# cvxopt/cvxopt

Hardware: NVIDIA H100
Metric: kkt_factor_solve_gflops_fp64 (higher is better)
Workload: dtype f64

## Files before the change

cvxopt_b200/csrc/chol.cu:

```cuda
#include "common.cuh"
#include <cstdlib>

namespace cvxb {

namespace {

constexpr int PB = 8;
constexpr int SP = 12;
constexpr int LDM = NB + 4;
constexpr int POTF2_SMEM = (NB * LDM + NB * SP + 4 * 80) * 8;

template <int PAT>
__device__ __forceinline__ void sym_update(double (&acc)[4][8][2], const double *Ma, const double *Mb) {
#pragma unroll 2
    for (int kk = 0; kk < NB / 4; ++kk) {
        double a[4], bfr[8];
#pragma unroll
        for (int cf = 0; cf < 4; ++cf) a[cf] = -Ma[cf * 8 + kk * 4 * LDM];
#pragma unroll
        for (int rf = 0; rf < 8; ++rf) bfr[rf] = Mb[rf * 8 + kk * 4 * LDM];
#pragma unroll
        for (int mf = 0; mf < 2; ++mf)
#pragma unroll
            for (int rf = 0; rf < 8; ++rf) {
                if (PAT == 1 && rf < 2 * mf) continue;
                if (PAT == 2 && rf < 4 + 2 * mf) continue;
                dmma16x8x4(acc[2 * mf][rf][0], acc[2 * mf][rf][1], acc[2 * mf + 1][rf][0], acc[2 * mf + 1][rf][1],
                           a[2 * mf], a[2 * mf + 1], bfr[rf]);
            }
    }
}

__global__ void __launch_bounds__(256, 1)
potf2_inv_kernel(double *A, long long lda, int jb, double *inv, double *invT, int *info, int joff,
                 long long sA, long long sInv, const double *Tprev, long long ldt,
                 const double *invprev, unsigned long long *trace) {
    extern __shared__ __align__(16) double sm[];
    if (trace && threadIdx.x == 0) {
        unsigned long long t; asm volatile("mov.u64 %0, %%globaltimer;" : "=l"(t)); trace[0] = t;
    }
#define CVXB_STAMP(SLOT)                                                                    \
    if (trace && threadIdx.x == 0) {                                                        \
        unsigned long long t_; asm volatile("mov.u64 %0, %%globaltimer;" : "=l"(t_));       \
        trace[8 * 2048 + (SLOT)] = t_;                                                      \
    }
    A += (long long)blockIdx.x * sA; inv += (long long)blockIdx.x * sInv;
    invT += (long long)blockIdx.x * sInv; info += blockIdx.x;
    double *M = sm;
    double *P = M + NB * LDM;
    double *Dw = P + NB * SP;
    const int tid = threadIdx.x, lane = tid & 31, warp = tid >> 5;
    const int role = (0x72640531 >> (warp * 4)) & 7;
    const int wr = role & 1, wc = role >> 1;
    const int g4 = lane >> 2, t4 = lane & 3;

    double acc[4][8][2];
    if (Tprev != nullptr) {
#pragma unroll
        for (int cf = 0; cf < 4; ++cf)
#pragma unroll
            for (int rf = 0; rf < 8; ++rf) acc[cf][rf][0] = acc[cf][rf][1] = 0.0;
        const int kkmax = (wc + 1) * 8;
        {
            const bool v16 = ((ldt & 1) == 0) && ((reinterpret_cast<uintptr_t>(Tprev) & 15) == 0);
            if (v16) {
                for (int q = tid; q < NB * NB / 2; q += 256) {
                    const int c = q >> 6, r = (q & 63) * 2;
                    const int nb = (r + 1 < jb) ? 16 : (r < jb ? 8 : 0);
                    cp_async16(M + r + c * LDM, nb ? Tprev + r + (long long)c * ldt : Tprev, nb);
                }
            } else {
                for (int q = tid; q < NB * NB; q += 256) {
                    const int c = q >> 7, r = q & 127;
                    cp_async8(M + r + c * LDM, (r < jb) ? Tprev + r + (long long)c * ldt : Tprev, (r < jb) ? 8 : 0);
                }
            }
            cp_async_commit();
        }
        const double *ip = invprev + (wc * 32 + g4) + t4 * NB;
        double a0[4];
#pragma unroll
        for (int cf = 0; cf < 4; ++cf) a0[cf] = ip[cf * 8];
        cp_async_wait<0>();
        __syncthreads();
        const double *tq = M + (wr * 64 + g4) + t4 * LDM;
#pragma unroll 2
        for (int kk = 0; kk < kkmax; ++kk) {
            double a[4], bfr[8];
#pragma unroll
            for (int cf = 0; cf < 4; ++cf) a[cf] = a0[cf];
            if (kk + 1 < kkmax) {
#pragma unroll
                for (int cf = 0; cf < 4; ++cf) a0[cf] = ip[cf * 8 + (kk + 1) * 4 * NB];
            }
#pragma unroll
            for (int rf = 0; rf < 8; ++rf) bfr[rf] = tq[rf * 8 + kk * 4 * LDM];
#pragma unroll
            for (int mf = 0; mf < 2; ++mf)
#pragma unroll
                for (int rf = 0; rf < 8; ++rf)
                    dmma16x8x4(acc[2 * mf][rf][0], acc[2 * mf][rf][1], acc[2 * mf + 1][rf][0],
                               acc[2 * mf + 1][rf][1], a[2 * mf], a[2 * mf + 1], bfr[rf]);
        }
        __syncthreads();
#pragma unroll
        for (int cf = 0; cf < 4; ++cf)
#pragma unroll
            for (int rf = 0; rf < 8; ++rf)
#pragma unroll
                for (int e = 0; e < 2; ++e)
                    M[(wr * 64 + rf * 8 + t4 * 2 + e) + (wc * 32 + cf * 8 + g4) * LDM] = acc[cf][rf][e];
    }
    CVXB_STAMP(0)
#pragma unroll
    for (int cf = 0; cf < 4; ++cf)
#pragma unroll
        for (int rf = 0; rf < 8; ++rf)
#pragma unroll
            for (int e = 0; e < 2; ++e) {
                const int r = wr * 64 + rf * 8 + t4 * 2 + e, c = wc * 32 + cf * 8 + g4;
                double v = (r == c) ? 1.0 : 0.0;
                if (r < jb && c < jb && r >= c) v = A[r + (long long)c * lda];
                acc[cf][rf][e] = v;
            }
    __syncthreads();
    CVXB_STAMP(4)
    if (Tprev != nullptr) {
        const int d = wc - 2 * wr;
        const double *Ma = M + (wc * 32 + g4) + t4 * LDM;
        const double *Mb = M + (wr * 64 + g4) + t4 * LDM;
        if (d < 0) sym_update<0>(acc, Ma, Mb);
        else if (d == 0) sym_update<1>(acc, Ma, Mb);
        else if (d == 1) sym_update<2>(acc, Ma, Mb);
        __syncthreads();
    }
    CVXB_STAMP(1)
#pragma unroll 1
    for (int t = 0; t < NB / PB; ++t) {
      {
        const int c0 = t * PB;
        if (wc == (t >> 2)) {
#define CVXB_PUBLISH(CF)                                                          \
    _Pragma("unroll") for (int rf = 0; rf < 8; ++rf)                              \
        _Pragma("unroll") for (int e = 0; e < 2; ++e)                             \
            P[(wr * 64 + rf * 8 + t4 * 2 + e) * SP + g4] = acc[CF][rf][e];
            switch (t & 3) {
                case 0: CVXB_PUBLISH(0) break;
                case 1: CVXB_PUBLISH(1) break;
                case 2: CVXB_PUBLISH(2) break;
                default: CVXB_PUBLISH(3) break;
            }
#undef CVXB_PUBLISH
        }
        __syncthreads();
        if (warp == 0 && lane == 0) {
            double a[PB][PB];
#pragma unroll
            for (int i = 0; i < PB; ++i)
#pragma unroll
                for (int k = 0; k <= i; ++k) a[i][k] = P[(c0 + i) * SP + k];
            bool bad = false;
#pragma unroll
            for (int j = 0; j < PB; ++j) {
                const double piv = a[j][j];
                if (!(piv > 0.0) && !bad) {
                    atomicCAS(info, 0, joff + c0 + j + 1);
                    bad = true;
                }
                const double rs = rsqrt(piv);
                a[j][j] = piv * rs;
                Dw[64 + j] = rs;
#pragma unroll
                for (int i = j + 1; i < PB; ++i) a[i][j] *= rs;
#pragma unroll
                for (int k = j + 1; k < PB; ++k)
#pragma unroll
                    for (int i = k; i < PB; ++i) a[i][k] -= a[i][j] * a[k][j];
            }
#pragma unroll
            for (int i = 0; i < PB; ++i)
#pragma unroll
                for (int k = 0; k < PB; ++k) Dw[i * 8 + k] = (k <= i) ? a[i][k] : 0.0;
        }
        if (warp < 4) asm volatile("bar.sync 1, 128;" ::: "memory");
        if (warp < 4) {
            const double *D = Dw;
            const int r = warp * 32 + lane;
            double x[PB];
            if (r >= c0 + PB) {
#pragma unroll
                for (int j = 0; j < PB; ++j) x[j] = P[r * SP + j];
#pragma unroll
                for (int j = 0; j < PB; ++j) {
                    double v = x[j];
#pragma unroll
                    for (int k = 0; k < j; ++k) v -= x[k] * D[j * 8 + k];
                    x[j] = v * D[64 + j];
                }
            } else if (r >= c0) {
#pragma unroll
                for (int j = 0; j < PB; ++j) x[j] = (j <= r - c0) ? D[(r - c0) * 8 + j] : 0.0;
            } else {
#pragma unroll
                for (int j = 0; j < PB; ++j) x[j] = 0.0;
            }
#pragma unroll
            for (int j = 0; j < PB; ++j) P[r * SP + j] = x[j];
        }
        __syncthreads();
        if (wr * 8 + 7 > t && wc * 4 + 3 > t) {
            double a[4][2], bfr[8][2];
#pragma unroll
            for (int kk = 0; kk < 2; ++kk) {
#pragma unroll
                for (int cf = 0; cf < 4; ++cf) a[cf][kk] = -P[(wc * 32 + cf * 8 + g4) * SP + kk * 4 + t4];
#pragma unroll
                for (int rf = 0; rf < 8; ++rf) bfr[rf][kk] = P[(wr * 64 + rf * 8 + g4) * SP + kk * 4 + t4];
            }
#pragma unroll
            for (int mf = 0; mf < 2; ++mf) {
                if (wc * 4 + 2 * mf + 1 <= t) continue;
#pragma unroll
                for (int rf = 0; rf < 8; ++rf) {
                    dmma16x8x4(acc[2 * mf][rf][0], acc[2 * mf][rf][1], acc[2 * mf + 1][rf][0], acc[2 * mf + 1][rf][1],
                               a[2 * mf][0], a[2 * mf + 1][0], bfr[rf][0]);
                    dmma16x8x4(acc[2 * mf][rf][0], acc[2 * mf][rf][1], acc[2 * mf + 1][rf][0], acc[2 * mf + 1][rf][1],
                               a[2 * mf][1], a[2 * mf + 1][1], bfr[rf][1]);
                }
            }
        }
        for (int e = tid; e < NB * PB; e += 256) {
            const int r = e & (NB - 1), j = e >> 7;
            const double v = P[r * SP + j];
            M[r + (c0 + j) * LDM] = v;
            if (r >= c0 + j && r < jb && c0 + j < jb) A[r + (long long)(c0 + j) * lda] = v;
        }
        __syncthreads();
      }
    }

    CVXB_STAMP(2)
    {
        const int blk = warp * 2 + (lane >> 4);
        const int j = lane & 15;
        const int o = blk * PB;
        double x[PB];
        if (j < PB) {
#pragma unroll
            for (int i = 0; i < PB; ++i) {
                double v = (i == j) ? 1.0 : 0.0;
#pragma unroll
                for (int k = 0; k < i; ++k)
                    if (k >= j) v -= M[(o + i) + (o + k) * LDM] * x[k];
                x[i] = (i >= j) ? v / M[(o + i) + (o + i) * LDM] : 0.0;
            }
        }
        __syncwarp();
        if (j < PB) {
#pragma unroll
            for (int i = 0; i < PB; ++i) M[(o + i) + (o + j) * LDM] = x[i];
        }
    }
    __syncthreads();
    for (int s = PB; s < NB; s <<= 1) {
        const int sb = s / PB;
        const int tp = sb * sb;
        const int ntiles = (NB / (2 * s)) * tp;
#pragma unroll 1
        for (int phase = 0; phase < 2; ++phase) {
            for (int base = warp * 4; base < ntiles; base += 32) {
                double c[4][2];
                int oo[4], ti[4], tj[4];
#pragma unroll
                for (int u = 0; u < 4; ++u) {
                    const int idx = min(base + u, ntiles - 1);
                    const int pr = idx / tp, loc = idx - pr * tp;
                    ti[u] = loc % sb; tj[u] = loc / sb; oo[u] = pr * 2 * s;
                    c[u][0] = c[u][1] = 0.0;
                }
                for (int kb = 0; kb < sb; ++kb) {
#pragma unroll
                    for (int u = 0; u < 4; ++u) {
                        const bool live = phase == 0 ? (kb >= tj[u]) : (kb <= ti[u]);
                        if (!live) continue;
                        const int o = oo[u];
#pragma unroll
                        for (int kk = 0; kk < 2; ++kk) {
                            const int k = kb * 8 + kk * 4 + t4;
                            double af, bf;
                            if (phase == 0) {
                                af = M[(o + s + ti[u] * 8 + g4) + (o + k) * LDM];
                                bf = M[(o + k) + (o + tj[u] * 8 + g4) * LDM];
                            } else {
                                af = M[(o + s + ti[u] * 8 + g4) + (o + s + k) * LDM];
                                bf = M[(o + k) + (o + s + tj[u] * 8 + g4) * LDM];
                            }
                            dmma(c[u][0], c[u][1], af, bf);
                        }
                    }
                }
#pragma unroll
                for (int u = 0; u < 4; ++u) {
                    if (base + u >= ntiles) continue;
                    const int o = oo[u];
                    if (phase == 0) {
                        M[(o + ti[u] * 8 + g4) + (o + s + tj[u] * 8 + t4 * 2) * LDM] = c[u][0];
                        M[(o + ti[u] * 8 + g4) + (o + s + tj[u] * 8 + t4 * 2 + 1) * LDM] = c[u][1];
                    } else {
                        M[(o + s + ti[u] * 8 + g4) + (o + tj[u] * 8 + t4 * 2) * LDM] = -c[u][0];
                        M[(o + s + ti[u] * 8 + g4) + (o + tj[u] * 8 + t4 * 2 + 1) * LDM] = -c[u][1];
                    }
                }
            }
            __syncthreads();
        }
    }
    CVXB_STAMP(3)
    for (int e = tid; e < NB * NB; e += 256) {
        int i = e & (NB - 1), k = e >> 7;
        inv[e] = (i >= k) ? M[i + k * LDM] : 0.0;
        invT[e] = (k >= i) ? M[k + i * LDM] : 0.0;
    }
    if (trace && threadIdx.x == 0) {
        unsigned long long t; asm volatile("mov.u64 %0, %%globaltimer;" : "=l"(t)); trace[1] = t;
    }
}

constexpr int TR_CH = 32;
constexpr int TR_R = 5;
constexpr int TRSV_SMEM = (TR_R * NB * TR_CH + 4 * NB + 32 * 129) * 8;

template <bool TRANS, bool VEC>
__global__ void __launch_bounds__(256, 1)
trsv_kernel(int n, const double *__restrict__ L, long long ldl, const double *__restrict__ inv,
            const double *__restrict__ invT, double *b, int *flags, int epoch, long long sL,
            long long sInv, long long sb) {
    extern __shared__ __align__(16) double sm[];
    {
        const long long pb = blockIdx.y;
        L += pb * sL; inv += pb * sInv; invT += pb * sInv; b += pb * sb;
        flags += pb * ((n + NB - 1) / NB);
    }
    double *ring = sm;
    double *xs = ring + TR_R * NB * TR_CH;
    double *part = xs + NB;
    double *tvec = part + 2 * NB;
    double *part2 = tvec + NB;
    const int nblk = (n + NB - 1) / NB;
    const int tid = threadIdx.x, lane = tid & 31, warp = tid >> 5;
    const int bi = TRANS ? (nblk - 1 - (int)blockIdx.x) : (int)blockIdx.x;
    const int i0 = bi * NB;
    const int ni = min(NB, n - i0);
    const int r = tid & (NB - 1), half = tid >> 7;

    double ireg[64];
    {
        const double *ip = (TRANS ? invT : inv) + (long long)bi * NB * NB + r + (long long)(half * 64) * NB;
#pragma unroll
        for (int k = 0; k < 64; ++k) ireg[k] = ip[k * NB];
    }

    const double bown = (tid < ni) ? b[i0 + tid] : 0.0;
    const int nb_dep = TRANS ? (nblk - 1 - bi) : bi;
    const int nchunks = nb_dep * (NB / TR_CH);
    auto issue = [&](int q) {
        const int jj = q / (NB / TR_CH), cc = q % (NB / TR_CH);
        const int j = TRANS ? (nblk - 1 - jj) : jj;
        double *dst = ring + (q % TR_R) * (NB * TR_CH);
        const double *src;
        int nrows, ncols;
        if (!TRANS) { src = L + i0 + (long long)(j * NB + cc * TR_CH) * ldl; nrows = ni; ncols = TR_CH; }
        else { src = L + (long long)j * NB + (long long)(i0 + cc * TR_CH) * ldl; nrows = min(NB, n - j * NB); ncols = min(TR_CH, ni - cc * TR_CH); }
        if (VEC) {
#pragma unroll
            for (int it = 0; it < 8; ++it) {
                const int e = tid + it * 256;
                const int c = e >> 6, rr = (e & 63) * 2;
                const int rem = nrows - rr;
                const int bytes = (c < ncols) ? (rem >= 2 ? 16 : (rem == 1 ? 8 : 0)) : 0;
                cp_async16(dst + c * NB + rr, bytes ? (src + rr + (long long)c * ldl) : L, bytes);
            }
        } else {
#pragma unroll
            for (int it = 0; it < 16; ++it) {
                const int e = tid + it * 256;
                const int c = e >> 7, rr = e & 127;
                const int bytes = (c < ncols && rr < nrows) ? 8 : 0;
                cp_async8(dst + c * NB + rr, bytes ? (src + rr + (long long)c * ldl) : L, bytes);
            }
        }
    };
#pragma unroll
    for (int q = 0; q < TR_R - 1; ++q) {
        if (q < nchunks) issue(q);
        cp_async_commit();
    }

    double acc = 0.0;
    double accc[16];
#pragma unroll
    for (int q = 0; q < 16; ++q) accc[q] = 0.0;

    for (int jj = 0; jj < nb_dep; ++jj) {
        const int j = TRANS ? (nblk - 1 - jj) : jj;
        if (tid == 0) while (ld_acquire(flags + j) != epoch) { }
        __syncthreads();
        if (tid < NB) xs[tid] = (j * NB + tid < n) ? __ldcg(b + j * NB + tid) : 0.0;
#pragma unroll
        for (int cc = 0; cc < NB / TR_CH; ++cc) {
            const int q = jj * (NB / TR_CH) + cc;
            cp_async_wait<TR_R - 2>();
            __syncthreads();
            {
                const int nq = q + TR_R - 1;
                if (nq < nchunks) issue(nq);
                cp_async_commit();
            }
            const double *ch = ring + (q % TR_R) * (NB * TR_CH);
            if (!TRANS) {
#pragma unroll
                for (int c = 0; c < 16; ++c)
                    acc += ch[(half * 16 + c) * NB + r] * xs[cc * TR_CH + half * 16 + c];
            } else {
#pragma unroll
                for (int qc = 0; qc < 4; ++qc) {
                    const double *col = ch + (warp * 4 + qc) * NB;
                    double a = 0.0;
#pragma unroll
                    for (int rr = 0; rr < 4; ++rr) a += col[lane + rr * 32] * xs[lane + rr * 32];
                    accc[cc * 4 + qc] += a;
                }
            }
        }
    }
    cp_async_wait<0>();
    __syncthreads();
    if (!TRANS) {
        part[half * NB + r] = acc;
        __syncthreads();
        if (tid < NB) tvec[tid] = (tid < ni) ? (bown - part[tid] - part[NB + tid]) : 0.0;
        __syncthreads();
    } else {
#pragma unroll
        for (int q = 0; q < 16; ++q) {
            const int c = (q >> 2) * TR_CH + warp * 4 + (q & 3);
            part2[lane * 129 + c] = accc[q];
        }
        __syncthreads();
        if (tid < NB) {
            double sacc = 0.0;
#pragma unroll 8
            for (int l = 0; l < 32; ++l) sacc += part2[l * 129 + tid];
            tvec[tid] = (tid < ni) ? (bown - sacc) : 0.0;
        }
        __syncthreads();
    }
    double a2 = 0.0;
#pragma unroll
    for (int k = 0; k < 64; ++k) a2 += ireg[k] * tvec[half * 64 + k];
    part[half * NB + r] = a2;
    __syncthreads();
    if (tid < ni) b[i0 + tid] = part[tid] + part[NB + tid];
    __threadfence();
    __syncthreads();
    if (tid == 0) st_release(flags + bi, epoch);
}

std::atomic<int> g_trsv_epoch{0};

}

int chol_work_create(CholWork &w) {
    int least = 0, greatest = 0;
    CVXB_CUDA(cudaDeviceGetStreamPriorityRange(&least, &greatest));
    CVXB_CUDA(cudaStreamCreateWithPriority(&w.panel_stream, cudaStreamNonBlocking, greatest));
    CVXB_CUDA(cudaStreamCreateWithPriority(&w.trsm_stream, cudaStreamNonBlocking, greatest));
    CVXB_CUDA(cudaStreamCreateWithPriority(&w.update_stream, cudaStreamNonBlocking, least));
    CVXB_CUDA(cudaEventCreateWithFlags(&w.ev_end_t, cudaEventDisableTiming));
    CVXB_CUDA(cudaEventCreateWithFlags(&w.ev_start, cudaEventDisableTiming));
    CVXB_CUDA(cudaEventCreateWithFlags(&w.ev_end_p, cudaEventDisableTiming));
    CVXB_CUDA(cudaEventCreateWithFlags(&w.ev_end_u, cudaEventDisableTiming));
    CVXB_TRY(w.d_info.alloc(1));
    CVXB_CUDA(cudaMemset(w.d_info.p, 0, sizeof(int)));
    CVXB_TRY(w.d_flags.alloc(4096));
    CVXB_CUDA(cudaMemset(w.d_flags.p, 0, 4096 * sizeof(int)));
    CVXB_TRY(w.splitk_ws.alloc(dmma_gemm_splitk_ws_doubles()));
    CVXB_CUDA(cudaFuncSetAttribute(potf2_inv_kernel, cudaFuncAttributeMaxDynamicSharedMemorySize,
                                   POTF2_SMEM));
    CVXB_CUDA(cudaFuncSetAttribute(trsv_kernel<true, true>, cudaFuncAttributeMaxDynamicSharedMemorySize, TRSV_SMEM));
    CVXB_CUDA(cudaFuncSetAttribute(trsv_kernel<true, false>, cudaFuncAttributeMaxDynamicSharedMemorySize, TRSV_SMEM));
    CVXB_CUDA(cudaFuncSetAttribute(trsv_kernel<false, true>, cudaFuncAttributeMaxDynamicSharedMemorySize, TRSV_SMEM));
    CVXB_CUDA(cudaFuncSetAttribute(trsv_kernel<false, false>, cudaFuncAttributeMaxDynamicSharedMemorySize, TRSV_SMEM));
    return 0;
}

CholWork::~CholWork() {
    for (cudaStream_t s : {panel_stream, update_stream, trsm_stream}) if (s) cudaStreamDestroy(s);
    for (auto &g : graphs) if (g.exec) cudaGraphExecDestroy(g.exec);
    for (cudaEvent_t e : {ev_end_t, ev_start, ev_end_p, ev_end_u}) if (e) cudaEventDestroy(e);
    for (auto *v : {&ev_dg, &ev_tr, &ev_c0, &ev_r})
        for (cudaEvent_t e : *v) cudaEventDestroy(e);
}

static int potrf_enqueue(int n, double *A, int lda, double *inv, CholWork &w, cudaStream_t st) {
    if (n <= 0) return 0;
    const int nblk = (n + NB - 1) / NB;
    if (w.panel_rows < n) {
        for (auto &g : w.graphs) if (g.exec) cudaGraphExecDestroy(g.exec);
        w.graphs.clear();
        for (DevBuf<double> &pb : w.panel) pb.reset();
        const int rows = (n + 1) & ~1;
        for (DevBuf<double> &pb : w.panel) CVXB_TRY(pb.alloc((size_t)rows * NB));
        w.panel_rows = rows;
    }
    while ((int)w.ev_dg.size() < nblk) {
        cudaEvent_t e[4];
        for (int i = 0; i < 4; ++i) CVXB_CUDA(cudaEventCreateWithFlags(&e[i], cudaEventDisableTiming));
        w.ev_dg.push_back(e[0]); w.ev_tr.push_back(e[1]); w.ev_c0.push_back(e[2]); w.ev_r.push_back(e[3]);
    }
    if (getenv("CVXB_TRACE") && !w.trace.p) CVXB_TRY(w.trace.alloc(8 * 4096));
    unsigned long long *trace = w.trace.p;
    if (trace) CVXB_CUDA(cudaMemsetAsync(trace, 0, 8 * 4096 * sizeof(unsigned long long), st));
    const int ldw = w.panel_rows;
    const int panel_tiles = NB / dmma_gemm_tile_cols();
    cudaStream_t D = w.panel_stream, T = w.trsm_stream, U = w.update_stream;
    CVXB_CUDA(cudaMemsetAsync(w.d_info.p, 0, sizeof(int), st));
    CVXB_CUDA(cudaEventRecord(w.ev_start, st));
    CVXB_CUDA(cudaStreamWaitEvent(D, w.ev_start, 0));
    CVXB_CUDA(cudaStreamWaitEvent(T, w.ev_start, 0));
    CVXB_CUDA(cudaStreamWaitEvent(U, w.ev_start, 0));
    int last_r = -1;
    int prev_r = -1;
    for (int jb = 0; jb < nblk; ++jb) {
        const int j = jb * NB;
        const int wj = (n - j < NB) ? (n - j) : NB;
        const int m = n - j - wj;
        double *Ajj = A + j + (long long)j * lda;
        double *invj = inv + (long long)jb * NB * NB;
        double *invTj = inv + (long long)(nblk + jb) * NB * NB;
        double *Wp = w.panel[jb & 1].p;
        if (jb >= 2) {
            CVXB_CUDA(cudaStreamWaitEvent(D, w.ev_c0[jb - 2], 0));
            const int rd = (last_r <= jb - 2) ? last_r : prev_r;
            if (rd >= 0) CVXB_CUDA(cudaStreamWaitEvent(D, w.ev_r[rd], 0));
        }
        const double *Tprev = jb > 0 ? A + j + (long long)(j - NB) * lda : nullptr;
        const double *invprev = jb > 0 ? inv + (long long)(jb - 1) * NB * NB : nullptr;
        potf2_inv_kernel<<<1, 256, POTF2_SMEM, D>>>(Ajj, lda, wj, invj, invTj, w.d_info.p, j, 0, 0, Tprev,
                                                     lda, invprev, trace ? trace + 8 * jb : nullptr);
        count_launch();
        CVXB_LAUNCH_CHECK();
        CVXB_CUDA(cudaEventRecord(w.ev_dg[jb], D));
        auto copy_back_prev = [&]() -> int {
            if (jb == 0) return 0;
            const int jp = j - NB, mp = n - j;
            CVXB_CUDA(cudaMemcpy2DAsync(A + j + (long long)jp * lda, (size_t)lda * sizeof(double),
                                        w.panel[(jb - 1) & 1].p, (size_t)ldw * sizeof(double),
                                        (size_t)mp * sizeof(double), NB, cudaMemcpyDeviceToDevice, T));
            return 0;
        };
        if (m <= 0) {
            CVXB_CUDA(cudaStreamWaitEvent(T, w.ev_dg[jb], 0));
            CVXB_TRY(copy_back_prev());
            break;
        }
        double *A21 = Ajj + wj;
        double *A22 = A21 + (long long)wj * lda;
        CVXB_CUDA(cudaStreamWaitEvent(T, w.ev_dg[jb], 0));
        if (prev_r >= 0) CVXB_CUDA(cudaStreamWaitEvent(T, w.ev_r[prev_r], 0));
        {
            GemmDesc g;
            g.M = m; g.N = wj; g.K = wj;
            g.X = A21; g.ldx = lda; g.x_kmajor = false;
            g.Y = invj; g.ldy = NB; g.y_kmajor = false;
            g.C = Wp; g.ldc = ldw;
            g.trace = trace ? trace + 8 * jb + 2 : nullptr;
            CVXB_TRY(dmma_gemm(g, T));
        }
        CVXB_CUDA(cudaEventRecord(w.ev_tr[jb], T));
        if (last_r >= 0) CVXB_CUDA(cudaStreamWaitEvent(T, w.ev_r[last_r], 0));
        const int wn = (m < NB) ? m : NB;
        if (m > wn) {
            GemmDesc c;
            c.M = m - wn; c.N = wn; c.K = wj;
            c.X = Wp + wn; c.Y = Wp;
            c.ldx = ldw; c.x_kmajor = false;
            c.ldy = ldw; c.y_kmajor = false;
            c.D = A22 + wn; c.ldd = lda; c.C = A22 + wn; c.ldc = lda;
            c.alpha = -1.0; c.beta = 1.0;
            c.trace = trace ? trace + 8 * jb + 4 : nullptr;
            CVXB_TRY(dmma_gemm(c, T));
        }
        CVXB_CUDA(cudaEventRecord(w.ev_c0[jb], T));
        CVXB_TRY(copy_back_prev());
        if (m > NB) {
            CVXB_CUDA(cudaStreamWaitEvent(U, w.ev_tr[jb], 0));
            GemmDesc u;
            u.M = m; u.N = m; u.K = wj;
            u.X = Wp; u.ldx = ldw; u.x_kmajor = false;
            u.Y = Wp; u.ldy = ldw; u.y_kmajor = false;
            u.D = A22; u.ldd = lda; u.C = A22; u.ldc = lda;
            u.alpha = -1.0; u.beta = 1.0; u.lower_only = true;
            u.ct_begin = panel_tiles; u.ct_end = 1 << 30;
            u.trace = trace ? trace + 8 * jb + 6 : nullptr;
            CVXB_TRY(dmma_gemm(u, U));
            CVXB_CUDA(cudaEventRecord(w.ev_r[jb], U));
            prev_r = last_r;
            last_r = jb;
        }
    }
    CVXB_CUDA(cudaEventRecord(w.ev_end_p, D));
    CVXB_CUDA(cudaEventRecord(w.ev_end_u, U));
    CVXB_CUDA(cudaEventRecord(w.ev_end_t, T));
    CVXB_CUDA(cudaStreamWaitEvent(st, w.ev_end_p, 0));
    CVXB_CUDA(cudaStreamWaitEvent(st, w.ev_end_u, 0));
    CVXB_CUDA(cudaStreamWaitEvent(st, w.ev_end_t, 0));
    return 0;
}

int potrf_lower(int n, double *A, int lda, double *inv, CholWork &w, cudaStream_t st) {
    if (n <= 0) return 0;
    if (w.graph_failed || n > 4096) return potrf_enqueue(n, A, lda, inv, w, st);
    CholWork::GraphEntry *ent = nullptr;
    for (auto &g : w.graphs)
        if (g.n == n && g.A == A && g.lda == lda && g.inv == inv) { ent = &g; break; }
    if (ent && ent->exec) {
        CVXB_CUDA(cudaGraphLaunch(ent->exec, st));
        count_launch(ent->launches);
        return 0;
    }
    if (!ent) {
        if (w.graphs.size() >= 4) {
            for (auto &g : w.graphs) if (g.exec) cudaGraphExecDestroy(g.exec);
            w.graphs.clear();
        }
        CholWork::GraphEntry g;
        g.n = n; g.A = A; g.lda = lda; g.inv = inv;
        w.graphs.push_back(g);
        return potrf_enqueue(n, A, lda, inv, w, st);
    }
    const unsigned long long l0 = g_launches.load();
    if (cudaStreamBeginCapture(st, cudaStreamCaptureModeRelaxed) != cudaSuccess) {
        cudaGetLastError();
        w.graph_failed = true;
        return potrf_enqueue(n, A, lda, inv, w, st);
    }
    const int rc = potrf_enqueue(n, A, lda, inv, w, st);
    cudaGraph_t graph = nullptr;
    const cudaError_t ce = cudaStreamEndCapture(st, &graph);
    const int captured = (int)(g_launches.load() - l0);
    g_launches.fetch_sub((unsigned long long)captured);
    if (rc != 0 || ce != cudaSuccess || !graph) {
        cudaGetLastError();
        if (graph) cudaGraphDestroy(graph);
        w.graph_failed = true;
        return potrf_enqueue(n, A, lda, inv, w, st);
    }
    cudaGraphExec_t exec = nullptr;
    if (cudaGraphInstantiate(&exec, graph, 0) != cudaSuccess || !exec) {
        cudaGetLastError();
        cudaGraphDestroy(graph);
        w.graph_failed = true;
        return potrf_enqueue(n, A, lda, inv, w, st);
    }
    cudaGraphDestroy(graph);
    ent->exec = exec;
    ent->launches = captured;
    CVXB_CUDA(cudaGraphLaunch(exec, st));
    count_launch(captured);
    return 0;
}

int trsv_lower(int n, const double *L, int ldl, const double *inv, double *b, bool trans,
               CholWork &w, cudaStream_t st, int batch, long long sL, long long sInv, long long sb) {
    if (n <= 0 || batch <= 0) return 0;
    const int nblk = (n + NB - 1) / NB;
    const size_t nflags = (size_t)nblk * batch;
    if (nflags > w.d_flags.n) {
        w.d_flags.reset();
        CVXB_TRY(w.d_flags.alloc(nflags));
        CVXB_CUDA(cudaMemset(w.d_flags.p, 0, nflags * sizeof(int)));
    }
    const int epoch = g_trsv_epoch.fetch_add(1) + 1;
    const double *invT = inv + (long long)nblk * NB * NB;
    const bool vec = ((uintptr_t)L % 16 == 0) && (ldl % 2 == 0) && (batch == 1 || sL % 2 == 0);
    dim3 grid(nblk, batch);
#define TRSV_LAUNCH(T, V) trsv_kernel<T, V><<<grid, 256, TRSV_SMEM, st>>>(n, L, ldl, inv, invT, b, w.d_flags.p, epoch, sL, sInv, sb)
    if (trans) { if (vec) TRSV_LAUNCH(true, true); else TRSV_LAUNCH(true, false); }
    else       { if (vec) TRSV_LAUNCH(false, true); else TRSV_LAUNCH(false, false); }
#undef TRSV_LAUNCH
    count_launch();
    CVXB_LAUNCH_CHECK();
    return 0;
}

int potrs_lower(int n, const double *L, int ldl, const double *inv, double *b, CholWork &w,
                cudaStream_t st, int batch, long long sL, long long sInv, long long sb) {
    CVXB_TRY(trsv_lower(n, L, ldl, inv, b, false, w, st, batch, sL, sInv, sb));
    CVXB_TRY(trsv_lower(n, L, ldl, inv, b, true, w, st, batch, sL, sInv, sb));
    return 0;
}

namespace {
__global__ void copy2d_batched_kernel(const double *src, long long lds, long long ssrc, double *dst,
                                      long long ldd, long long sdst, int rows, int cols) {
    const long long pb = blockIdx.z;
    const int r = blockIdx.x * blockDim.x + threadIdx.x, c = blockIdx.y;
    if (r < rows && c < cols) dst[pb * sdst + r + (long long)c * ldd] = src[pb * ssrc + r + (long long)c * lds];
}
}

int potrf_lower_batched(int n, double *A, int lda, long long sA, double *inv, long long sInv,
                        int batch, int *d_info, double *panel, int ldw, cudaStream_t st) {
    if (n <= 0 || batch <= 0) return 0;
    const int nblk = (n + NB - 1) / NB;
    CVXB_CUDA(cudaMemsetAsync(d_info, 0, (size_t)batch * sizeof(int), st));
    const long long sW = (long long)ldw * NB;
    for (int jb = 0; jb < nblk; ++jb) {
        const int j = jb * NB;
        const int wj = (n - j < NB) ? (n - j) : NB;
        const int m = n - j - wj;
        double *Ajj = A + j + (long long)j * lda;
        double *invj = inv + (long long)jb * NB * NB;
        double *invTj = inv + (long long)(nblk + jb) * NB * NB;
        potf2_inv_kernel<<<batch, 256, POTF2_SMEM, st>>>(Ajj, lda, wj, invj, invTj, d_info, j, sA, sInv, nullptr, 0,
                                                        nullptr, nullptr);
        count_launch();
        CVXB_LAUNCH_CHECK();
        if (m <= 0) break;
        double *A21 = Ajj + wj;
        double *A22 = A21 + (long long)wj * lda;
        GemmDesc g;
        g.M = m; g.N = wj; g.K = wj;
        g.X = A21; g.ldx = lda; g.x_kmajor = false; g.sX = sA;
        g.Y = invj; g.ldy = NB; g.y_kmajor = false; g.sY = sInv;
        g.C = panel; g.ldc = ldw; g.sC = sW; g.batch = batch;
        CVXB_TRY(dmma_gemm(g, st));
        GemmDesc u;
        u.M = m; u.N = m; u.K = wj;
        u.X = panel; u.ldx = ldw; u.x_kmajor = false; u.sX = sW;
        u.Y = panel; u.ldy = ldw; u.y_kmajor = false; u.sY = sW;
        u.D = A22; u.ldd = lda; u.sD = sA; u.C = A22; u.ldc = lda; u.sC = sA;
        u.alpha = -1.0; u.beta = 1.0; u.lower_only = true; u.batch = batch;
        CVXB_TRY(dmma_gemm(u, st));
        dim3 cg((m + 255) / 256, wj, batch);
        copy2d_batched_kernel<<<cg, 256, 0, st>>>(panel, ldw, sW, A21, lda, sA, m, wj);
        count_launch();
        CVXB_LAUNCH_CHECK();
    }
    return 0;
}

}
```

cvxopt_b200/csrc/common.cuh:

```cuda
#pragma once
#include <cuda_runtime.h>
#include <cstdio>
#include <cstdint>
#include <cstring>
#include <string>
#include <vector>
#include <atomic>
#include <mutex>
#include "../../include/cvxopt_b200.h"

namespace cvxb {

void set_error(const char *fmt, ...);
extern std::atomic<unsigned long long> g_launches;
inline void count_launch(int n = 1) { g_launches.fetch_add((unsigned long long)n, std::memory_order_relaxed); }

struct DeviceOnce {
    std::atomic<unsigned long long> done{0};
    unsigned long long pending() {
        int d = 0;
        cudaGetDevice(&d);
        const unsigned long long bit = 1ull << (d & 63);
        return (done.load(std::memory_order_acquire) & bit) ? 0ull : bit;
    }
    void mark(unsigned long long bit) { done.fetch_or(bit, std::memory_order_release); }
};

#define CVXB_CUDA(expr)                                                            \
    do {                                                                           \
        cudaError_t _e = (expr);                                                   \
        if (_e != cudaSuccess) {                                                   \
            cvxb::set_error("%s:%d: %s -> %s", __FILE__, __LINE__, #expr,          \
                            cudaGetErrorString(_e));                               \
            return CVXB_E_CUDA;                                                    \
        }                                                                          \
    } while (0)

#define CVXB_TRY(expr)                                                             \
    do {                                                                           \
        int _r = (expr);                                                           \
        if (_r != 0) return _r;                                                    \
    } while (0)

#define CVXB_LAUNCH_CHECK()                                                        \
    do {                                                                           \
        cudaError_t _e = cudaGetLastError();                                       \
        if (_e != cudaSuccess) {                                                   \
            cvxb::set_error("%s:%d: kernel launch -> %s", __FILE__, __LINE__,      \
                            cudaGetErrorString(_e));                               \
            return CVXB_E_CUDA;                                                    \
        }                                                                          \
    } while (0)

cudaError_t tmp_malloc_bytes(void **p, size_t bytes);
void tmp_free(void *p);
void tmp_cache_release();
template <class T> inline cudaError_t tmp_malloc(T **p, size_t bytes) { return tmp_malloc_bytes(reinterpret_cast<void **>(p), bytes); }

template <class T> struct Scratch {
    T *p = nullptr;
    Scratch() = default;
    Scratch(const Scratch &) = delete;
    Scratch &operator=(const Scratch &) = delete;
    ~Scratch() { tmp_free(p); }
    int alloc(size_t n) {
        CVXB_CUDA(tmp_malloc(&p, (n ? n : 1) * sizeof(T)));
        return 0;
    }
};

struct Staged {
    double *dev = nullptr, *host = nullptr; size_t n = 0; bool owned = false;
    Staged() = default;
    Staged(const Staged &) = delete;
    Staged &operator=(const Staged &) = delete;
    ~Staged() { if (owned) tmp_free(dev); }
    int in(const double *src, size_t count, int space, cudaStream_t st, bool upload = true) {
        n = count; host = const_cast<double *>(src);
        if (space == CVXB_DEVICE) { dev = host; return 0; }
        CVXB_CUDA(tmp_malloc(&dev, (n ? n : 1) * sizeof(double)));
        owned = true;
        if (n && upload) CVXB_CUDA(cudaMemcpyAsync(dev, src, n * sizeof(double), cudaMemcpyHostToDevice, st));
        return 0;
    }
    int out(cudaStream_t st) {
        if (owned && n) CVXB_CUDA(cudaMemcpyAsync(host, dev, n * sizeof(double), cudaMemcpyDeviceToHost, st));
        return 0;
    }
};

extern std::atomic<unsigned long long> g_device_bytes;

template <class T> struct DevBuf {
    T *p = nullptr;
    size_t n = 0;
    DevBuf() = default;
    DevBuf(const DevBuf &) = delete;
    DevBuf &operator=(const DevBuf &) = delete;
    DevBuf(DevBuf &&o) noexcept : p(o.p), n(o.n) { o.p = nullptr; o.n = 0; }
    DevBuf &operator=(DevBuf &&o) noexcept {
        if (this != &o) { reset(); p = o.p; n = o.n; o.p = nullptr; o.n = 0; }
        return *this;
    }
    ~DevBuf() { reset(); }
    cudaError_t try_alloc(size_t count) {
        reset();
        const size_t bytes = count * sizeof(T);
        cudaError_t e = cudaMalloc(&p, bytes);
        if (e == cudaErrorMemoryAllocation) { cudaGetLastError(); tmp_cache_release(); e = cudaMalloc(&p, bytes); }
        if (e != cudaSuccess) { cudaGetLastError(); p = nullptr; return e; }
        n = count;
        g_device_bytes.fetch_add(bytes, std::memory_order_relaxed);
        return cudaSuccess;
    }
    int alloc(size_t count) {
        const cudaError_t e = try_alloc(count);
        if (e == cudaSuccess) return 0;
        set_error("cudaMalloc(%zu bytes) -> %s", count * sizeof(T), cudaGetErrorString(e));
        return e == cudaErrorMemoryAllocation ? CVXB_E_NOMEM : CVXB_E_CUDA;
    }
    void reset() {
        if (!p) return;
        cudaFree(p);
        g_device_bytes.fetch_sub(n * sizeof(T), std::memory_order_relaxed);
        p = nullptr;
        n = 0;
    }
};

bool coop_launch_fits(const void *kernel, int threads, long long ctas);

constexpr int kNumSMs = 132;
constexpr int NB = 128;

#ifdef __CUDACC__
__device__ __forceinline__ void dmma(double &d0, double &d1, double a, double b) {
    asm volatile("mma.sync.aligned.m8n8k4.row.col.f64.f64.f64.f64 {%0,%1}, {%2}, {%3}, {%0,%1};"
                 : "+d"(d0), "+d"(d1)
                 : "d"(a), "d"(b));
}
__device__ __forceinline__ void dmma16x8x4(double &d0, double &d1, double &d2, double &d3, double a0, double a1,
                                           double b) {
    asm volatile("mma.sync.aligned.m16n8k4.row.col.f64.f64.f64.f64 {%0,%1,%2,%3}, {%4,%5}, {%6}, {%0,%1,%2,%3};"
                 : "+d"(d0), "+d"(d1), "+d"(d2), "+d"(d3)
                 : "d"(a0), "d"(a1), "d"(b));
}

__device__ __forceinline__ uint32_t smem_u32(const void *p) {
    return (uint32_t)__cvta_generic_to_shared(p);
}
__device__ __forceinline__ void cp_async16(void *smem, const void *gmem, int src_bytes) {
    asm volatile("cp.async.cg.shared.global [%0], [%1], 16, %2;" ::"r"(smem_u32(smem)), "l"(gmem),
                 "r"(src_bytes));
}
__device__ __forceinline__ void cp_async8(void *smem, const void *gmem, int src_bytes) {
    asm volatile("cp.async.ca.shared.global [%0], [%1], 8, %2;" ::"r"(smem_u32(smem)), "l"(gmem),
                 "r"(src_bytes));
}
__device__ __forceinline__ void cp_async_commit() { asm volatile("cp.async.commit_group;"); }
template <int N>
__device__ __forceinline__ void cp_async_wait() {
    asm volatile("cp.async.wait_group %0;" ::"n"(N));
}

__device__ __forceinline__ void mbar_init(uint64_t *bar, int count) {
    asm volatile("mbarrier.init.shared::cta.b64 [%0], %1;" ::"r"(smem_u32(bar)), "r"(count));
}
__device__ __forceinline__ void mbar_expect_tx(uint64_t *bar, uint32_t bytes) {
    asm volatile("mbarrier.arrive.expect_tx.shared::cta.b64 _, [%0], %1;" ::"r"(smem_u32(bar)), "r"(bytes)
                 : "memory");
}
__device__ __forceinline__ void mbar_arrive(uint64_t *bar) {
    asm volatile("mbarrier.arrive.shared::cta.b64 _, [%0];" ::"r"(smem_u32(bar)) : "memory");
}
__device__ __forceinline__ void mbar_wait(uint64_t *bar, uint32_t parity) {
    asm volatile(
        "{\n\t.reg .pred p;\n\t"
        "WAIT_%=:\n\t"
        "mbarrier.try_wait.parity.shared::cta.b64 p, [%0], %1;\n\t"
        "@p bra DONE_%=;\n\t"
        "bra WAIT_%=;\n\t"
        "DONE_%=:\n\t}" ::"r"(smem_u32(bar)), "r"(parity)
        : "memory");
}
__device__ __forceinline__ void bulk_g2s(void *dst, const void *src, uint32_t bytes, uint64_t *bar) {
    asm volatile(
        "cp.async.bulk.shared::cluster.global.mbarrier::complete_tx::bytes [%0], [%1], %2, [%3];"
        ::"r"(smem_u32(dst)), "l"(src), "r"(bytes), "r"(smem_u32(bar))
        : "memory");
}
__device__ __forceinline__ void tma_load_1d(void *dst, const void *map, int c0, uint64_t *bar) {
    asm volatile(
        "cp.async.bulk.tensor.1d.shared::cluster.global.tile.mbarrier::complete_tx::bytes [%0], [%1, {%2}], [%3];"
        ::"r"(smem_u32(dst)), "l"(map), "r"(c0), "r"(smem_u32(bar))
        : "memory");
}
__device__ __forceinline__ void tma_load_2d(void *dst, const void *map, int c0, int c1, uint64_t *bar) {
    asm volatile(
        "cp.async.bulk.tensor.2d.shared::cluster.global.tile.mbarrier::complete_tx::bytes [%0], [%1, {%2, %3}], [%4];"
        ::"r"(smem_u32(dst)), "l"(map), "r"(c0), "r"(c1), "r"(smem_u32(bar))
        : "memory");
}

__device__ __forceinline__ double warp_sum(double v) {
#pragma unroll
    for (int o = 16; o > 0; o >>= 1) v += __shfl_xor_sync(0xffffffffu, v, o);
    return v;
}
__device__ __forceinline__ double warp_min(double v) {
#pragma unroll
    for (int o = 16; o > 0; o >>= 1) v = fmin(v, __shfl_xor_sync(0xffffffffu, v, o));
    return v;
}
__device__ __forceinline__ double block_sum(double v, double *sh) {
    v = warp_sum(v);
    const int lane = threadIdx.x & 31, warp = threadIdx.x >> 5;
    __syncthreads();
    if (lane == 0) sh[warp] = v;
    __syncthreads();
    double t = (threadIdx.x < (blockDim.x >> 5)) ? sh[threadIdx.x] : 0.0;
    if (warp == 0) t = warp_sum(t);
    if (threadIdx.x == 0) sh[0] = t;
    __syncthreads();
    const double r = sh[0];
    __syncthreads();
    return r;
}
__device__ __forceinline__ double block_min(double v, double *sh) {
    v = warp_min(v);
    const int lane = threadIdx.x & 31, warp = threadIdx.x >> 5;
    __syncthreads();
    if (lane == 0) sh[warp] = v;
    __syncthreads();
    double t = (threadIdx.x < (blockDim.x >> 5)) ? sh[threadIdx.x] : INFINITY;
    if (warp == 0) t = warp_min(t);
    if (threadIdx.x == 0) sh[0] = t;
    __syncthreads();
    const double r = sh[0];
    __syncthreads();
    return r;
}
__device__ __forceinline__ int ld_acquire(const int *p) {
    int v;
    asm volatile("ld.acquire.gpu.global.s32 %0, [%1];" : "=r"(v) : "l"(p) : "memory");
    return v;
}
__device__ __forceinline__ void st_release(int *p, int v) {
    asm volatile("st.release.gpu.global.s32 [%0], %1;" ::"l"(p), "r"(v) : "memory");
}
#endif

struct GemmDesc {
    int M = 0, N = 0, K = 0;
    const double *X = nullptr; int ldx = 0; bool x_kmajor = false;
    const double *Y = nullptr; int ldy = 0; bool y_kmajor = false;
    const double *w = nullptr;
    const double *D = nullptr; int ldd = 0;
    double *C = nullptr; int ldc = 0;
    double alpha = 1.0, beta = 0.0;
    bool lower_only = false;
    int ct_begin = 0, ct_end = 1 << 30;
    int batch = 1;
    long long sX = 0, sY = 0, sW = 0, sD = 0, sC = 0;
    double *splitk_ws = nullptr;
    unsigned long long *trace = nullptr;
};
int dmma_gemm(const GemmDesc &g, cudaStream_t st);
size_t dmma_gemm_splitk_ws_doubles();
int dmma_gemm_tile_cols();

size_t ozaki_workspace_bytes(int n, int m, int S);
int ozaki_mode();
bool ozaki_use(int mode, int n, int m, DevBuf<char> &work);
void ozaki_time_mma(cudaEvent_t a, cudaEvent_t b);
int ozaki_syrk(int n, int m, const double *A, long long lda, const double *d, const double *D,
               long long ldd, double beta, double *C, long long ldc, int S, int layout, void *work,
               cudaStream_t st);

struct CholWork {
    cudaStream_t panel_stream = nullptr;
    cudaStream_t trsm_stream = nullptr;
    cudaStream_t update_stream = nullptr;
    cudaEvent_t ev_end_t = nullptr;
    std::vector<cudaEvent_t> ev_dg, ev_tr, ev_c0, ev_r;
    DevBuf<unsigned long long> trace;
    struct GraphEntry {
        int n = 0, lda = 0, launches = 0;
        const void *A = nullptr, *inv = nullptr;
        cudaGraphExec_t exec = nullptr;
    };
    std::vector<GraphEntry> graphs;
    bool graph_failed = false;
    cudaEvent_t ev_start = nullptr, ev_end_p = nullptr, ev_end_u = nullptr;
    DevBuf<int> d_info;
    DevBuf<int> d_flags;
    DevBuf<double> splitk_ws;
    DevBuf<double> panel[2];
    int panel_rows = 0;
    ~CholWork();
};
int chol_work_create(CholWork &w);
int potrf_lower(int n, double *A, int lda, double *inv, CholWork &w, cudaStream_t st);
int potrs_lower(int n, const double *L, int ldl, const double *inv, double *b, CholWork &w,
                cudaStream_t st, int batch = 1, long long sL = 0, long long sInv = 0,
                long long sb = 0);
int trsv_lower(int n, const double *L, int ldl, const double *inv, double *b, bool trans,
               CholWork &w, cudaStream_t st, int batch = 1, long long sL = 0, long long sInv = 0,
               long long sb = 0);
int potrf_lower_batched(int n, double *A, int lda, long long sA, double *inv, long long sInv,
                        int batch, int *d_info, double *panel, int ldw, cudaStream_t st);
int trsm_lower_left(int n, const double *L, long long ldl, const double *inv, double *B, long long ldb, int ncols,
                    cudaStream_t st, int batch = 1, long long sL = 0, long long sInv = 0, long long sB = 0);

int check_device(int device);

struct CallCtx {
    cudaStream_t st = nullptr;
    CholWork *cw = nullptr;
    std::unique_lock<std::mutex> lock;
    int acquire(int device);
};

}
```

Baseline: 38600.

## Aggregate trailing updates over groups of panels with a separate near-update stream

Restructures the blocked Cholesky trailing update. Near columns within the current group of four panels are updated per panel on a new high-priority stream. Far columns receive one GEMM with K=4*NB, using panels transposed into a group buffer. This replaces one rank-NB lower-triangular update per panel over the whole trailing matrix, aiming for larger-K GEMMs with better reuse and fewer full-matrix passes. The cost is a transpose kernel per panel, extra group buffers, and more complex cross-stream event dependencies that could serialize or introduce races.

```diff
diff --git a/cvxopt_b200/csrc/chol.cu b/cvxopt_b200/csrc/chol.cu
--- a/cvxopt_b200/csrc/chol.cu
+++ b/cvxopt_b200/csrc/chol.cu
@@ -9,6 +9,7 @@
 constexpr int SP = 12;
 constexpr int LDM = NB + 4;
 constexpr int POTF2_SMEM = (NB * LDM + NB * SP + 4 * 80) * 8;
+constexpr int kGroup = 4;
 
 template <int PAT>
 __device__ __forceinline__ void sym_update(double (&acc)[4][8][2], const double *Ma, const double *Mb) {
@@ -468,6 +469,19 @@
 
 std::atomic<int> g_trsv_epoch{0};
 
+__global__ void __launch_bounds__(256)
+transpose_panel_kernel(const double *__restrict__ W, long long ldw, int rows, double *__restrict__ WT, long long ldt) {
+    __shared__ double t[32][33];
+    const int r0 = blockIdx.x * 32, k0 = blockIdx.y * 32, tx = threadIdx.x, ty = threadIdx.y;
+#pragma unroll
+    for (int i = ty; i < 32; i += 8)
+        if (r0 + tx < rows) t[i][tx] = W[r0 + tx + (long long)(k0 + i) * ldw];
+    __syncthreads();
+#pragma unroll
+    for (int i = ty; i < 32; i += 8)
+        if (r0 + i < rows) WT[k0 + tx + (long long)(r0 + i) * ldt] = t[tx][i];
+}
+
 }
 
 int chol_work_create(CholWork &w) {
@@ -476,7 +490,9 @@
     CVXB_CUDA(cudaStreamCreateWithPriority(&w.panel_stream, cudaStreamNonBlocking, greatest));
     CVXB_CUDA(cudaStreamCreateWithPriority(&w.trsm_stream, cudaStreamNonBlocking, greatest));
     CVXB_CUDA(cudaStreamCreateWithPriority(&w.update_stream, cudaStreamNonBlocking, least));
+    CVXB_CUDA(cudaStreamCreateWithPriority(&w.near_stream, cudaStreamNonBlocking, greatest));
     CVXB_CUDA(cudaEventCreateWithFlags(&w.ev_end_t, cudaEventDisableTiming));
+    CVXB_CUDA(cudaEventCreateWithFlags(&w.ev_end_n, cudaEventDisableTiming));
     CVXB_CUDA(cudaEventCreateWithFlags(&w.ev_start, cudaEventDisableTiming));
     CVXB_CUDA(cudaEventCreateWithFlags(&w.ev_end_p, cudaEventDisableTiming));
     CVXB_CUDA(cudaEventCreateWithFlags(&w.ev_end_u, cudaEventDisableTiming));
@@ -495,10 +511,10 @@
 }
 
 CholWork::~CholWork() {
-    for (cudaStream_t s : {panel_stream, update_stream, trsm_stream}) if (s) cudaStreamDestroy(s);
+    for (cudaStream_t s : {panel_stream, update_stream, trsm_stream, near_stream}) if (s) cudaStreamDestroy(s);
     for (auto &g : graphs) if (g.exec) cudaGraphExecDestroy(g.exec);
-    for (cudaEvent_t e : {ev_end_t, ev_start, ev_end_p, ev_end_u}) if (e) cudaEventDestroy(e);
-    for (auto *v : {&ev_dg, &ev_tr, &ev_c0, &ev_r})
+    for (cudaEvent_t e : {ev_end_t, ev_end_n, ev_start, ev_end_p, ev_end_u}) if (e) cudaEventDestroy(e);
+    for (auto *v : {&ev_dg, &ev_tr, &ev_c0, &ev_na, &ev_nb, &ev_n})
         for (cudaEvent_t e : *v) cudaEventDestroy(e);
 }
 
@@ -509,28 +525,46 @@
         for (auto &g : w.graphs) if (g.exec) cudaGraphExecDestroy(g.exec);
         w.graphs.clear();
         for (DevBuf<double> &pb : w.panel) pb.reset();
+        for (DevBuf<double> &gb : w.group) gb.reset();
         const int rows = (n + 1) & ~1;
         for (DevBuf<double> &pb : w.panel) CVXB_TRY(pb.alloc((size_t)rows * NB));
+        for (DevBuf<double> &gb : w.group) CVXB_TRY(gb.alloc((size_t)rows * kGroup * NB));
         w.panel_rows = rows;
     }
     while ((int)w.ev_dg.size() < nblk) {
-        cudaEvent_t e[4];
-        for (int i = 0; i < 4; ++i) CVXB_CUDA(cudaEventCreateWithFlags(&e[i], cudaEventDisableTiming));
-        w.ev_dg.push_back(e[0]); w.ev_tr.push_back(e[1]); w.ev_c0.push_back(e[2]); w.ev_r.push_back(e[3]);
+        cudaEvent_t e[6];
+        for (int i = 0; i < 6; ++i) CVXB_CUDA(cudaEventCreateWithFlags(&e[i], cudaEventDisableTiming));
+        w.ev_dg.push_back(e[0]); w.ev_tr.push_back(e[1]); w.ev_c0.push_back(e[2]);
+        w.ev_na.push_back(e[3]); w.ev_nb.push_back(e[4]); w.ev_n.push_back(e[5]);
     }
     if (getenv("CVXB_TRACE") && !w.trace.p) CVXB_TRY(w.trace.alloc(8 * 4096));
     unsigned long long *trace = w.trace.p;
     if (trace) CVXB_CUDA(cudaMemsetAsync(trace, 0, 8 * 4096 * sizeof(unsigned long long), st));
     const int ldw = w.panel_rows;
-    const int panel_tiles = NB / dmma_gemm_tile_cols();
-    cudaStream_t D = w.panel_stream, T = w.trsm_stream, U = w.update_stream;
+    const int ldg = kGroup * NB;
+    cudaStream_t D = w.panel_stream, T = w.trsm_stream, U = w.update_stream, N = w.near_stream;
     CVXB_CUDA(cudaMemsetAsync(w.d_info.p, 0, sizeof(int), st));
     CVXB_CUDA(cudaEventRecord(w.ev_start, st));
-    CVXB_CUDA(cudaStreamWaitEvent(D, w.ev_start, 0));
-    CVXB_CUDA(cudaStreamWaitEvent(T, w.ev_start, 0));
-    CVXB_CUDA(cudaStreamWaitEvent(U, w.ev_start, 0));
-    int last_r = -1;
-    int prev_r = -1;
+    for (cudaStream_t s : {D, T, U, N}) CVXB_CUDA(cudaStreamWaitEvent(s, w.ev_start, 0));
+    auto update = [&](int lo, int hi, const double *X, int ldx, bool kmajor, int K, unsigned long long *tr,
+                      cudaStream_t s) -> int {
+        double *Acc = A + (long long)lo * NB * (1 + (long long)lda);
+        GemmDesc u;
+        u.M = n - lo * NB; u.N = (hi * NB < n ? hi * NB : n) - lo * NB; u.K = K;
+        u.X = X; u.ldx = ldx; u.x_kmajor = kmajor;
+        u.Y = X; u.ldy = ldx; u.y_kmajor = kmajor;
+        u.D = Acc; u.ldd = lda; u.C = Acc; u.ldc = lda;
+        u.alpha = -1.0; u.beta = 1.0; u.lower_only = true;
+        u.trace = tr;
+        return dmma_gemm(u, s);
+    };
+    auto wait_col = [&](cudaStream_t s, int c) -> int {
+        const int p = c - 2, g0 = kGroup * (c / kGroup);
+        if (p < 0) return 0;
+        if (p >= g0) CVXB_CUDA(cudaStreamWaitEvent(s, w.ev_na[p], 0));
+        if (g0 > 0) CVXB_CUDA(cudaStreamWaitEvent(s, w.ev_nb[p < g0 - 1 ? p : g0 - 1], 0));
+        return 0;
+    };
     for (int jb = 0; jb < nblk; ++jb) {
         const int j = jb * NB;
         const int wj = (n - j < NB) ? (n - j) : NB;
@@ -539,11 +573,8 @@
         double *invj = inv + (long long)jb * NB * NB;
         double *invTj = inv + (long long)(nblk + jb) * NB * NB;
         double *Wp = w.panel[jb & 1].p;
-        if (jb >= 2) {
-            CVXB_CUDA(cudaStreamWaitEvent(D, w.ev_c0[jb - 2], 0));
-            const int rd = (last_r <= jb - 2) ? last_r : prev_r;
-            if (rd >= 0) CVXB_CUDA(cudaStreamWaitEvent(D, w.ev_r[rd], 0));
-        }
+        if (jb >= 2) CVXB_CUDA(cudaStreamWaitEvent(D, w.ev_c0[jb - 2], 0));
+        CVXB_TRY(wait_col(D, jb));
         const double *Tprev = jb > 0 ? A + j + (long long)(j - NB) * lda : nullptr;
         const double *invprev = jb > 0 ? inv + (long long)(jb - 1) * NB * NB : nullptr;
         potf2_inv_kernel<<<1, 256, POTF2_SMEM, D>>>(Ajj, lda, wj, invj, invTj, w.d_info.p, j, 0, 0, Tprev,
@@ -567,7 +598,7 @@
         double *A21 = Ajj + wj;
         double *A22 = A21 + (long long)wj * lda;
         CVXB_CUDA(cudaStreamWaitEvent(T, w.ev_dg[jb], 0));
-        if (prev_r >= 0) CVXB_CUDA(cudaStreamWaitEvent(T, w.ev_r[prev_r], 0));
+        if (jb >= 2) CVXB_CUDA(cudaStreamWaitEvent(T, w.ev_n[jb - 2], 0));
         {
             GemmDesc g;
             g.M = m; g.N = wj; g.K = wj;
@@ -578,7 +609,7 @@
             CVXB_TRY(dmma_gemm(g, T));
         }
         CVXB_CUDA(cudaEventRecord(w.ev_tr[jb], T));
-        if (last_r >= 0) CVXB_CUDA(cudaStreamWaitEvent(T, w.ev_r[last_r], 0));
+        CVXB_TRY(wait_col(T, jb + 1));
         const int wn = (m < NB) ? m : NB;
         if (m > wn) {
             GemmDesc c;
@@ -593,28 +624,39 @@
         }
         CVXB_CUDA(cudaEventRecord(w.ev_c0[jb], T));
         CVXB_TRY(copy_back_prev());
-        if (m > NB) {
-            CVXB_CUDA(cudaStreamWaitEvent(U, w.ev_tr[jb], 0));
-            GemmDesc u;
-            u.M = m; u.N = m; u.K = wj;
-            u.X = Wp; u.ldx = ldw; u.x_kmajor = false;
-            u.Y = Wp; u.ldy = ldw; u.y_kmajor = false;
-            u.D = A22; u.ldd = lda; u.C = A22; u.ldc = lda;
-            u.alpha = -1.0; u.beta = 1.0; u.lower_only = true;
-            u.ct_begin = panel_tiles; u.ct_end = 1 << 30;
-            u.trace = trace ? trace + 8 * jb + 6 : nullptr;
-            CVXB_TRY(dmma_gemm(u, U));
-            CVXB_CUDA(cudaEventRecord(w.ev_r[jb], U));
-            prev_r = last_r;
-            last_r = jb;
+        const int q = jb / kGroup, s = jb % kGroup, gq = kGroup * (q + 1);
+        double *Wg = w.group[q & 1].p;
+        unsigned long long *tr_near = trace ? trace + 8 * jb + 6 : nullptr;
+        CVXB_CUDA(cudaStreamWaitEvent(N, w.ev_tr[jb], 0));
+        if (s == 0 && jb > 0) CVXB_CUDA(cudaStreamWaitEvent(N, w.ev_nb[jb - 1], 0));
+        {
+            const int lo = jb + 2, hi = gq < nblk ? gq : nblk;
+            if (lo < hi) CVXB_TRY(update(lo, hi, Wp + (lo - jb - 1) * NB, ldw, false, NB, tr_near, N));
+        }
+        CVXB_CUDA(cudaEventRecord(w.ev_na[jb], N));
+        if (gq < nblk) {
+            const int rows = n - gq * NB;
+            transpose_panel_kernel<<<dim3((rows + 31) / 32, NB / 32), dim3(32, 8), 0, N>>>(
+                Wp + (gq - jb - 1) * NB, ldw, rows, Wg + s * NB, ldg);
+            count_launch();
+            CVXB_LAUNCH_CHECK();
+        }
+        CVXB_CUDA(cudaEventRecord(w.ev_n[jb], N));
+        if (gq < nblk) {
+            CVXB_CUDA(cudaStreamWaitEvent(U, w.ev_n[jb], 0));
+            const int lo = gq > jb + 2 ? gq : jb + 2, hi = gq + kGroup < nblk ? gq + kGroup : nblk;
+            if (lo < hi) CVXB_TRY(update(lo, hi, Wg + s * NB + (long long)(lo - gq) * NB * ldg, ldg, true, NB, tr_near, U));
+            CVXB_CUDA(cudaEventRecord(w.ev_nb[jb], U));
+            if (s == kGroup - 1 && gq + kGroup < nblk)
+                CVXB_TRY(update(gq + kGroup, nblk, Wg + (long long)kGroup * NB * ldg, ldg, true, kGroup * NB,
+                                trace ? trace + 8 * 2048 + 8 * jb + 5 : nullptr, U));
         }
     }
     CVXB_CUDA(cudaEventRecord(w.ev_end_p, D));
     CVXB_CUDA(cudaEventRecord(w.ev_end_u, U));
     CVXB_CUDA(cudaEventRecord(w.ev_end_t, T));
-    CVXB_CUDA(cudaStreamWaitEvent(st, w.ev_end_p, 0));
-    CVXB_CUDA(cudaStreamWaitEvent(st, w.ev_end_u, 0));
-    CVXB_CUDA(cudaStreamWaitEvent(st, w.ev_end_t, 0));
+    CVXB_CUDA(cudaEventRecord(w.ev_end_n, N));
+    for (cudaEvent_t e : {w.ev_end_p, w.ev_end_u, w.ev_end_t, w.ev_end_n}) CVXB_CUDA(cudaStreamWaitEvent(st, e, 0));
     return 0;
 }
 
diff --git a/cvxopt_b200/csrc/common.cuh b/cvxopt_b200/csrc/common.cuh
--- a/cvxopt_b200/csrc/common.cuh
+++ b/cvxopt_b200/csrc/common.cuh
@@ -281,8 +281,9 @@
     cudaStream_t panel_stream = nullptr;
     cudaStream_t trsm_stream = nullptr;
     cudaStream_t update_stream = nullptr;
-    cudaEvent_t ev_end_t = nullptr;
-    std::vector<cudaEvent_t> ev_dg, ev_tr, ev_c0, ev_r;
+    cudaStream_t near_stream = nullptr;
+    cudaEvent_t ev_end_t = nullptr, ev_end_n = nullptr;
+    std::vector<cudaEvent_t> ev_dg, ev_tr, ev_c0, ev_na, ev_nb, ev_n;
     DevBuf<unsigned long long> trace;
     struct GraphEntry {
         int n = 0, lda = 0, launches = 0;
@@ -296,6 +297,7 @@
     DevBuf<int> d_flags;
     DevBuf<double> splitk_ws;
     DevBuf<double> panel[2];
+    DevBuf<double> group[2];
     int panel_rows = 0;
     ~CholWork();
 };
```

Result: faster. 40690, median of 6 (+5.4%).
